# kursawe/OpticalFlow

Measured on AMD Instinct MI355X. Metric: frame-pairs/sec, higher is better.
Workload: dtype f64; 1 GPU; 1024x1024x256 synthetic translating texture (seed 1), speed_alpha=1, remodelling_alpha=1e4, rtol=1e-06, all 255 pairs solved to the stopping rule; frames_per_gpu=256, pairs_in_flight=255, levels=9, coarse_stencils=float8, vcycle_vectors=coarse_float32, w_cycle_level=1, w_cycle_visits=3, warm_start_stride=3, allgather=False, gather_chunks=1, converged=True

## Files before the change

opticalflow_amd/csrc/vof.hip:

```cpp
#include "vof_device.hpp"
#include "vof_sweep0r.hpp"
#include "vof_sweep0p.hpp"
#include "vof_direct.hpp"
#include "vof_boxflow.hpp"
#include "vof_boxsweep.hpp"
#include "vof_blursweep.hpp"
#include "vof_liushen.hpp"
#include "../../include/vof.h"

#include <fcntl.h>
#include <unistd.h>

#include <algorithm>
#include <atomic>
#include <chrono>
#include <cmath>
#include <condition_variable>
#include <cstdio>
#include <cstdlib>
#include <cstring>
#include <mutex>
#include <string>
#include <thread>
#include <vector>
// ... 72 lines not shown
    char* sw_aux = nullptr;
    size_t sw_aux_bytes = 0;
    bool bf_lds_set = false;
    bool bl_lds_set = false;
    bool ls_lds_set = false;
    double* tex_tab = nullptr;
    size_t tex_cap = 0;
    double* gm_V = nullptr;
    GmresState* gm_state = nullptr;
    double* gm_partials = nullptr;
    int* gm_cycle = nullptr;
    int gm_m = 0;
    long long gmres_pairs = 0;
    struct Alloc { void* raw; char* user; size_t bytes; const char* name; int line; };
    std::vector<Alloc> allocs;
    int c_bytes_per_point = 0;
    size_t bytes = 0;
    std::string err;
    const double* frames = nullptr;
    int npairs = 0;
    vof_params prm;
    int cfmt = 0;
    bool fused = true;
    bool fold_stored = false;
    bool direct_on = false;
    int dir_cap = 0;
    double *dir_T = nullptr, *dir_tabs = nullptr, *dir_W = nullptr, *dir_r = nullptr, *dir_y = nullptr, *dir_x = nullptr, *dir_t = nullptr;
    int *dir_ipiv = nullptr, *dir_info = nullptr;
    double *dir_R = nullptr, *dir_C = nullptr, *dir_D = nullptr;
    int dir_ld = 0;
    long long direct_pairs = 0;
    bool fuse_rr = true;
    bool fuse_b = true;
    long sweep0r_min_blocks = 512;
    int tail_first = -1;
    size_t tail_lds = 0;
    TailArgs tail;
    int tail_key[6] = {-9, -9, -9, -9, -9, -9};
    bool prof = false;
    int prof_kid = -1, prof_level = -1;
    std::vector<ProfRec> recs;
    std::vector<hipEvent_t> free_events;
    long long prof_dropped = 0;
    double prof_ms[VOF_K_COUNT][16];
    long long prof_n[VOF_K_COUNT][16];
    long long prof_units[VOF_K_COUNT][16];
    double prof_bytes[VOF_K_COUNT][16];
    double prof_moved[VOF_K_COUNT][16];
    int cur_units = 0;
    int dbg_sync = 0;
    long long dbg_seq = 0;
    std::string dbg_fault;
    int dbg_fd = -1;
    bool dbg_canary = false;
    bool dbg_alloc_log = false;
    bool dbg_poison = false;
    size_t part_per_pair = 0;
    vof_ctx* lane_parent = nullptr;
    int lane_lo = 0, lane_slots = 0;
    int dir_ok = -1;
    hipStream_t lane_stream[MAX_LANES] = {};
    hipEvent_t lane_ev[MAX_LANES][2] = {};
    hipEvent_t ev_fork = nullptr;
    hipEvent_t group_ev[MAX_LANES * MAX_LANE_GROUPS] = {};
};

// ... 262 lines not shown
    }
}

int pick_band_height(int rows, int nx, int units) {
    const long blocks128 = (long)nx * ((rows + 127) / 128) * std::max(1, units);
    const int cap = blocks128 < 768 ? 32 : (blocks128 < 1536 ? 64 : 128);
    const int nb = (rows + cap - 1) / cap;
    return std::max(2, (((rows + nb - 1) / nb + 1) / 2) * 2);
}

struct ApplyGrid { int TI, nblk; dim3 grid; };
ApplyGrid apply_grid(const vof_ctx* c, int np) {
    const Level& lv = c->L[0];
    int TI = pick_band_height(lv.ni, (lv.nj + AP_OUT - 1) / AP_OUT, c->cur_units);
    ApplyGrid g;
    g.TI = TI;
    g.grid = dim3((lv.nj + AP_OUT - 1) / AP_OUT, (lv.ni + TI - 1) / TI, np);
    g.nblk = g.grid.x * g.grid.y;
    return g;
}

template <typename XT, typename BT, typename YT>
void apply_fine_t(vof_ctx* c, const XT* x, const BT* b, YT* y, int mode, int np, const int* active,
                  const double* dotvec = nullptr, int want_yy = 0, YT* ycopy = nullptr) {
    Level& lv = c->L[0];
    const double bytes = (8.0 + 3.0 * sizeof(XT) + ((y ? 3.0 : 0.0) + (ycopy ? 3.0 : 0.0)) * sizeof(YT) + (mode ? 3.0 * sizeof(BT) : 0.0) +
                          (dotvec ? 24.0 : 0.0)) * lv.npts;
    Prof p(c, VOF_K_APPLY0, 0, bytes);
    ApplyGrid ag = apply_grid(c, np);
    double* part = (dotvec || want_yy) ? c->partials : nullptr;
    if (mode)
        k_stream_apply0<1, XT, BT, YT><<<ag.grid, AP_THREADS, 0, c->stream>>>(
            c->frames, frame_stride(c), c->Nj, lv.ni, lv.nj, ag.TI, c->prm.speed_alpha, c->prm.remodelling_alpha,
            c->prm.reference_quirks, x, b, y, dotvec, want_yy, part, ag.nblk, active, c->pp, ycopy);
    else
        k_stream_apply0<0, XT, BT, YT><<<ag.grid, AP_THREADS, 0, c->stream>>>(
            c->frames, frame_stride(c), c->Nj, lv.ni, lv.nj, ag.TI, c->prm.speed_alpha, c->prm.remodelling_alpha,
            c->prm.reference_quirks, x, b, y, dotvec, want_yy, part, ag.nblk, active, c->pp, ycopy);
}

template <typename VT>
void apply_stored_t(vof_ctx* c, int l, const VT* x, const VT* b, VT* y, int mode, int np, const int* active) {
    Level& lv = c->L[l];
    dim3 g = grid2d(lv.ni, lv.nj, np);
    Prof p(c, VOF_K_RESIDUAL, l, (coef_bytes(c, l) + (mode ? 9.0 : 6.0) * sizeof(VT)) * lv.npts);
    if (mode) CDISPATCH(c, l, (k_apply<CT, 1, VT><<<g, blk2d, 0, c->stream>>>((const CW*)lv.C, lv.ni, lv.nj, x, b, y, active)));
    else CDISPATCH(c, l, (k_apply<CT, 0, VT><<<g, blk2d, 0, c->stream>>>((const CW*)lv.C, lv.ni, lv.nj, x, b, y, active)));
}

template <typename VT>
void apply_level_t(vof_ctx* c, int l, const VT* x, const VT* b, VT* y, int mode, int np, const int* active) {
    if (l == 0 && c->L[0].C == nullptr) apply_fine_t<VT, VT, VT>(c, x, b, y, mode, np, active);
    else apply_stored_t<VT>(c, l, x, b, y, mode, np, active);
}

int krylov_apply(vof_ctx* c, const void* y, double* out, int np, const int* active, const double* dotvec = nullptr,
                 int want_yy = 0) {
    if (c->L[0].C) { apply_stored_t<double>(c, 0, (const double*)y, nullptr, out, 0, np, active); return 0; }
    if (c->vfloat || c->h32) apply_fine_t<float, double, double>(c, (const float*)y, nullptr, out, 0, np, active, dotvec, want_yy);
    else apply_fine_t<double, double, double>(c, (const double*)y, nullptr, out, 0, np, active, dotvec, want_yy);
    return (dotvec || want_yy) ? apply_grid(c, np).nblk : 0;
}
inline bool residual_copy_ok(const vof_ctx* c) { return !c->L[0].C; }
int residual_d(vof_ctx* c, const double* x, const double* b, double* out, int np, const int* active, int want_norm = 0,
               double* out2 = nullptr) {
    if (!out && !(want_norm && !c->L[0].C)) return 0;
    if (c->L[0].C) { apply_stored_t<double>(c, 0, x, b, out, 1, np, active); return 0; }
    apply_fine_t<double, double, double>(c, x, b, out, 1, np, active, nullptr, want_norm ? 1 : 0, out2);
    return want_norm ? apply_grid(c, np).nblk : 0;
}

template <typename VT>
void restrict_level_t(vof_ctx* c, int l, const VT* fine, VT* coarse, int np, const int* active) {
    Level &f = c->L[l], &k = c->L[l + 1];
    Prof p(c, VOF_K_RESTRICT, l, 3.0 * sizeof(VT) * (f.npts + k.npts));
    k_restrict<VT><<<grid2d(k.ni, k.nj, np), blk2d, 0, c->stream>>>(fine, f.ni, f.nj, coarse, k.ni, k.nj, active);
}

template <typename VT, typename CVT = VT>
void resrestrict_fine_t(vof_ctx* c, const VT* x, const VT* b, CVT* bc, int np, const int* active) {
    Level &f = c->L[0], &k = c->L[1];
    int TI = pick_band_height(f.ni, (k.nj + RR_CO - 1) / RR_CO, c->cur_units);
    dim3 g((k.nj + RR_CO - 1) / RR_CO, (k.ni + TI / 2 - 1) / (TI / 2), np);
    Prof p(c, VOF_K_APPLY0, 0, (8.0 + 6.0 * sizeof(VT)) * f.npts + 3.0 * sizeof(CVT) * k.npts);
    k_stream_resrestrict0<VT, VT, CVT><<<g, AP_THREADS, 0, c->stream>>>(
        c->frames, frame_stride(c), c->Nj, f.ni, f.nj, TI, c->prm.speed_alpha, c->prm.remodelling_alpha,
        c->prm.reference_quirks, x, b, bc, k.ni, k.nj, active, c->pp);
}

inline double resu_coef_bytes(const vof_ctx* c) {
    return c->cfmt == 3 ? 12.0 * 4 : (c->cfmt == 2 ? 18.5 * 4 : (c->cfmt == 1 ? 36.0 * 4 : 36.0 * 8));
}
template <typename VT>
void resrestrict_u_t(vof_ctx* c, int l, const VT* x_new, const VT* x_old, VT* bc, int np, const int* active) {
    Level &f = c->L[l], &k = c->L[l + 1];
    const double vs = sizeof(VT);
    const double algo = (coef_bytes(c, l) + 9.0 * vs) * f.npts + 3.0 * vs * (f.npts + k.npts);
    const double moved = (resu_coef_bytes(c) + (x_old ? 6.0 : 3.0) * vs) * f.npts + 3.0 * vs * k.npts;
    Prof p(c, VOF_K_RESIDUAL, l, algo, moved);
    dim3 g(1, (k.ni + BY - 1) / BY, np);
    CDISPATCH(c, l, {
        if (x_old) k_resrestrict_u<CT, VT, true><<<g, blk2d, 0, c->stream>>>((const CW*)f.C, f.ni, f.nj, x_new, x_old, bc, k.ni, k.nj, active);
// ... 900 lines not shown
        if (rq.table) {
            HIPCHK(hipMemcpyAsync(c->pp_buf, rq.table, (size_t)np * sizeof(PairParam), hipMemcpyHostToDevice, c->stream));
            c->pp = c->pp_buf;
        }
        if (rq.guess) {
            HIPCHK(hipMemcpyAsync(c->warm_src, rq.guess, (size_t)np * sizeof(int), hipMemcpyHostToDevice, c->stream));
            guess_src = c->warm_src;
        }
    }
    c->direct_on = rq.direct;
    struct MaxItGuard { vof_params& p; int saved; ~MaxItGuard() { p.max_iterations = saved; } } max_it_guard{c->prm, c->prm.max_iterations};
    constexpr int MG_ATTEMPT_CAP = 150;
    if (P.preconditioner == 2 && !c->direct_on && c->L.size() > 1 && P.max_iterations > MG_ATTEMPT_CAP && 3 * c->L[0].nj <= 3100 &&
        direct_ok_for_fallback(c))
        c->prm.max_iterations = MG_ATTEMPT_CAP;
    if (stats) HIPCHK(hipEventRecord(c->ev_batch[0], c->stream));
    c->vfloat = (P.vcycle_precision == 1 || P.vcycle_precision == 2) && c->fused && c->L.size() > 1 && !c->direct_on;
    c->vcoarse32 = P.vcycle_precision == 3 && !c->direct_on;
    c->h32 = false;
    if (c->direct_on) {
        if (np > c->dir_cap) { c->err = "batch larger than the direct preconditioner's buffers"; return -1; }
        c->frames = frames_dev;
        c->npairs = np;
        c->cur_units = np;
        if (int rc = direct_setup(c, np)) return rc;
        c->direct_pairs += np;
    } else if (int rc = setup_batch(c, frames_dev, np)) return rc;
    Level& f = c->L[0];
    const size_t len = 3 * f.npts;
    hipStream_t s = c->stream;
    double sx = P.delta_t / P.delta_x;
    const bool zero_guess = !guess_src && (P.initial_v_x == 0.0 && P.initial_v_y == 0.0 && P.initial_remodelling == 0.0);
    double* rh = c->krh;
    {
        Prof p(c, VOF_K_RHS, 0);
        k_rhs_norm<<<rgrid(c, np), RBLK, 0, s>>>(frames_dev, frame_stride(c), c->Nj, f.ni, f.nj, c->kb, zero_guess ? c->kr : nullptr,
                                                c->partials, c->pp);
    }
    { Prof p(c, VOF_K_VECTOR, 0); k_scalar<S_BNORM><<<np, 64, 0, s>>>(c->sc, c->partials, c->nblk, c->active, P.rtol, P.max_iterations); }
    int nb0 = c->nblk;
    if (zero_guess) {
        HIPCHK(hipMemsetAsync(c->kx, 0, (size_t)np * len * sizeof(double), s));
        rh = c->kb;
    } else {
        if (guess_src) {
            Prof p(c, VOF_K_VECTOR, 0, 16.0 * len);
            k_gather_guess<<<rgrid(c, np), RBLK, 0, s>>>(c->kx, c->warm_x, guess_src, len, f.npts, P.initial_v_x * sx, P.initial_v_y * sx,
                                                        P.initial_remodelling);
        } else {
            Prof p(c, VOF_K_VECTOR, 0); k_fill<<<dim3(c->nblk, np), 256, 0, s>>>(c->kx, f.npts, P.initial_v_x * sx, P.initial_v_y * sx, P.initial_remodelling);
        }
        const bool two = residual_copy_ok(c);
        nb0 = residual_d(c, c->kx, c->kb, c->kr, np, nullptr, 1, two ? c->krh : nullptr);
        if (!two) HIPCHK(hipMemcpyAsync(c->krh, c->kr, (size_t)np * len * sizeof(double), hipMemcpyDeviceToDevice, s));
    }
    if (!nb0) {
        Prof p(c, VOF_K_REDUCE, 0); k_dot2<<<rgrid(c, np), RBLK, 0, s>>>(c->kr, c->kr, nullptr, nullptr, len, c->partials, nullptr);
        nb0 = c->nblk;
    }
    { Prof p(c, VOF_K_VECTOR, 0); k_scalar<S_R0><<<np, 64, 0, s>>>(c->sc, c->partials, nb0, c->active, P.rtol, P.max_iterations); }

    const int bicg_limit = P.krylov_method == 1 ? 0 : (P.krylov_method == 2 ? std::min(P.max_iterations, P.fallback_after) : P.max_iterations);
    int it_total = 0;
    auto bicg_loop = [&](int limit) -> int {
    bool ran_on_r = false;
    for (int it = 0; it < limit; ++it, ++it_total) {
        HIPCHK(hipMemcpyAsync(c->h_active, c->active, np * sizeof(int), hipMemcpyDeviceToHost, s));
        HIPCHK(hipStreamSynchronize(s));
        int nact = 0;
        for (int k = 0; k < np; ++k) nact += c->h_active[k] != 0;
        if (nact == 0) break;
        if (it_total == AUTO_F64_AFTER) { if (P.vcycle_precision == 2) c->vfloat = false; c->vcoarse32 = false; }
        c->cur_units = nact;
        c->h32 = handoff32_ok(c);
        const int* act = c->active;
        void* vrhs_p = c->vfloat ? (void*)c->b32 : (void*)c->kp;
        void* vrhs_s = c->vfloat ? (void*)c->b32 : (void*)c->kr;
        const double vsz = (c->vfloat || c->h32) ? 4.0 : 8.0;
        const bool on_r = it == 0 && !c->vfloat;
        const bool fold_b = fold_b_usable(c);
        auto cycle_ok = [c](const CycleIO& io, const char* which) {
            if (io.failed) c->h32 = false;
            else if (io.bf_mode && !io.bf_done) c->err = std::string("folded vector update (") + which + "): not consumed by the cycle";
            else return true;
            return false;
        };
        CycleIO io_p, io_s;
        if (on_r) vrhs_p = (void*)c->kr;
        else if (fold_b && it > 0) {
            const double* p_old = (it == 1 && ran_on_r) ? rh : c->kp;
            io_p.bf = S0BSrc{c->kr, c->kv, p_old, c->kt, c->sc, nullptr};
            io_p.bf_mode = 2;
            std::swap(c->kp, c->kt);
// ... 17 lines not shown
            std::swap(c->kr, c->kt);
            vrhs_s = (void*)c->kr;
        } else {
        { Prof p(c, VOF_K_VECTOR, 0, 8.0 * len * 3 + (c->vfloat ? 4.0 * len : 0.0));
          VDISPATCH(c, (k_update_s<VT><<<rgrid(c, np), RBLK, 0, s>>>(c->kr, c->kv, len, c->sc, c->partials, act, c->vfloat ? (VT*)c->b32 : (VT*)nullptr))); }
        { Prof p(c, VOF_K_VECTOR, 0); k_scalar<S_S><<<np, 64, 0, s>>>(c->sc, c->partials, c->nblk, c->active, P.rtol, P.max_iterations); }
        { Prof p(c, VOF_K_VECTOR, 0);
          YDISPATCH(c, (k_fix_half<VT><<<dim3(64, np), RBLK, 0, s>>>(c->kx, (const VT*)c->ky, len, c->sc)));
          k_clear_half<<<(np + 255) / 256, 256, 0, s>>>(c->sc, np); }
        }
        io_s.trail = S0Trail{c->kt, c->kr, 1, c->partials};
        vcycle(c, &c->kz, vrhs_s, np, act, io_s);
        if (!cycle_ok(io_s, "s")) return -1;
        int nb2 = io_s.trail_nblk ? io_s.trail_nblk : krylov_apply(c, c->kz, c->kt, np, act, c->kr, 1);
        if (!nb2) { Prof p(c, VOF_K_REDUCE, 0, 16.0 * len); k_dot2<<<rgrid(c, np), RBLK, 0, s>>>(c->kt, c->kr, c->kt, c->kt, len, c->partials, act); nb2 = c->nblk; }
        { Prof p(c, VOF_K_VECTOR, 0); k_scalar<S_OMEGA><<<np, 64, 0, s>>>(c->sc, c->partials, nb2, c->active, P.rtol, P.max_iterations); }
        { Prof p(c, VOF_K_VECTOR, 0, 8.0 * len * 6 + 2.0 * vsz * len);
          YDISPATCH(c, (k_update_xr<VT><<<rgrid(c, np), RBLK, 0, s>>>(c->kx, (const VT*)c->ky, (const VT*)c->kz, c->kr, c->kt, rh, len, c->sc, c->partials, act))); }
        { Prof p(c, VOF_K_VECTOR, 0); k_scalar<S_R><<<np, 64, 0, s>>>(c->sc, c->partials, c->nblk, c->active, P.rtol, P.max_iterations); }
    }
    c->h32 = false;
    return 0;
    };
    if (int rc = bicg_loop(bicg_limit)) return rc;
    auto independent_residual = [&](bool keep) -> int {
        c->cur_units = np;
        int nb3 = keep ? 0 : residual_d(c, c->kx, c->kb, nullptr, np, nullptr, 1);
        if (!nb3) nb3 = residual_d(c, c->kx, c->kb, c->kt, np, nullptr, 1);
        if (!nb3) { Prof p(c, VOF_K_REDUCE, 0); k_dot2<<<rgrid(c, np), RBLK, 0, s>>>(c->kt, c->kt, nullptr, nullptr, len, c->partials, nullptr); nb3 = c->nblk; }
        { Prof p(c, VOF_K_VECTOR, 0); k_scalar<S_FINAL><<<np, 64, 0, s>>>(c->sc, c->partials, nb3, c->active, P.rtol, P.max_iterations); }
        HIPCHK(hipGetLastError());
        return 0;
    };
    if (int rc = independent_residual(false)) return rc;
    if (bicg_limit > 0) {
        for (int round = 0; round < 3; ++round) {
            { Prof p(c, VOF_K_VECTOR, 0); k_bicg_restart<<<(np + 63) / 64, 64, 0, s>>>(c->sc, c->active, np, P.max_iterations); }
            int nact = count_active(c, np);
            if (nact < 0) { c->err = "stream synchronize failed"; return -2; }
            if (nact == 0) break;
            if (int rc = independent_residual(true)) return rc;
            c->cur_units = nact;
            rh = c->krh;
            { Prof p(c, VOF_K_VECTOR, 0, 8.0 * len * 3);
              k_restart_vectors<<<rgrid(c, np), RBLK, 0, s>>>(c->kr, rh, c->kt, len, c->active); }
            if (int rc = bicg_loop(std::min(bicg_limit, 8))) return rc;
            if (int rc = independent_residual(false)) return rc;
        }
    }
    if (P.krylov_method != 0) {
        int handed_over = 0;
        if (int rc = gmres_phase(c, np, &handed_over)) return rc;
        if (handed_over)
            if (int rc = independent_residual(false)) return rc;
    }
    { Prof p(c, VOF_K_FINALIZE, 0);
      k_finalize_functionals<<<rgrid(c, np), RBLK, 0, s>>>(frames_dev, frame_stride(c), f.ni, f.nj, P.speed_alpha, P.remodelling_alpha,
                                                           P.reference_quirks, c->kx, P.delta_x / P.delta_t, rq.vx, rq.vy, rq.gm, rq.speed,
                                                           c->partials, c->pp);
      k_sum3<<<np, 64, 0, s>>>(c->partials, c->nblk, c->func3); }
    HIPCHK(hipGetLastError());
    if (stats) {
        HIPCHK(hipMemcpyAsync(c->h_sc, c->sc, np * sizeof(PairScalars), hipMemcpyDeviceToHost, s));
        HIPCHK(hipMemcpyAsync(c->h_func3, c->func3, np * 3 * sizeof(double), hipMemcpyDeviceToHost, s));
        HIPCHK(hipEventRecord(c->ev_batch[1], s));
        HIPCHK(hipStreamSynchronize(s));
        float batch_ms = 0.f;
        HIPCHK(hipEventElapsedTime(&batch_ms, c->ev_batch[0], c->ev_batch[1]));
        for (int k = 0; k < np; ++k) {
            const PairScalars& q = c->h_sc[k];
            stats[k].iterations = q.iterations;
            stats[k].relative_residual = q.bnorm2 > 0 ? std::sqrt(q.rnorm2 / q.bnorm2) : 0.0;
            stats[k].converged = (q.rnorm2 <= q.tol2) ? 1 : 0;
            stats[k].L1_functional = c->h_func3[3 * k];
            stats[k].speed_functional = c->h_func3[3 * k + 1];
            stats[k].remodelling_functional = c->h_func3[3 * k + 2];
            stats[k].batch_ms = batch_ms;
            stats[k].batch_pairs = np;
            stats[k].reserved = 0;
        }
    }
    return 0;
}

int check_params(vof_ctx* c, const vof_params* p) {
    if (!p) { c->err = "params is NULL"; return -1; }
    if (p->struct_size != sizeof(vof_params) || p->abi_version != VOF_VERSION) {
        char buf[256];
        snprintf(buf, sizeof buf, "vof_params ABI mismatch: caller has struct_size %u / version %u, library has %zu / %d "
                 "(fill the struct with vof_default_params(p, sizeof *p) of the matching include/vof.h)",
                 p->struct_size, p->abi_version, sizeof(vof_params), VOF_VERSION);
        c->err = buf;
        return -4;
// ... 131 lines not shown
    for (hipEvent_t e : c->group_ev) if (e) hipEventDestroy(e);
    if (c->own_stream && c->stream) hipStreamDestroy(c->stream);
    delete c;
}

static int create_impl(vof_ctx* c, int device_id, int n_i, int n_j, int B, void* stream) {
    if (n_i < 4 || n_j < 4) { c->err = "image must be at least 4x4 (the mirror boundary rows need N >= 4)"; return -1; }
    if (B < 1) { c->err = "max_pairs_in_flight must be >= 1"; return -1; }
    int ndev = 0;
    HIPCHK(hipGetDeviceCount(&ndev));
    if (device_id < 0 || device_id >= ndev) { c->err = "no such HIP device"; return -1; }
    HIPCHK(hipSetDevice(device_id));
    c->device = device_id;
    c->Ni = n_i; c->Nj = n_j; c->B = B;
    if (stream) { c->stream = (hipStream_t)stream; c->own_stream = false; }
    else { HIPCHK(hipStreamCreate(&c->stream)); c->own_stream = true; }
    memset(c->prof_ms, 0, sizeof c->prof_ms);
    memset(c->prof_n, 0, sizeof c->prof_n);
    memset(c->prof_units, 0, sizeof c->prof_units);
    memset(c->prof_bytes, 0, sizeof c->prof_bytes);
    memset(c->prof_moved, 0, sizeof c->prof_moved);
    vof_default_params(&c->prm, sizeof c->prm);
    if (const char* e = getenv("VOF_DEBUG_SYNC")) c->dbg_sync = atoi(e);
    if (const char* e = getenv("VOF_DEBUG_CANARY")) c->dbg_canary = e[0] != '0';
    if (const char* e = getenv("VOF_DEBUG_ALLOC_LOG")) c->dbg_alloc_log = e[0] != '0';
    if (const char* e = getenv("VOF_DEBUG_POISON")) c->dbg_poison = e[0] != '0';
    if (c->dbg_sync)
        if (const char* e = getenv("VOF_DEBUG_SYNC_FILE")) c->dbg_fd = open(e, O_WRONLY | O_CREAT, 0644);
    if (const char* e = getenv("VOF_FOLD_STORED")) c->fold_stored = e[0] != '0';
    if (const char* e = getenv("VOF_L0_HANDOFF")) c->l0_handoff = e[0] != '0';
    if (const char* e = getenv("VOF_SWEEP0R_MIN_BLOCKS")) c->sweep0r_min_blocks = atol(e);
    if (const char* e = getenv("VOF_FUSE_B")) c->fuse_b = e[0] != '0';
    if (const char* e = getenv("VOF_FUSE_RR")) c->fuse_rr = e[0] != '0';
    Level l0; l0.ni = n_i - 2; l0.nj = n_j - 2; l0.npts = (size_t)l0.ni * l0.nj;
    c->L.push_back(l0);
    while (std::max(c->L.back().ni, c->L.back().nj) > COARSEST_MAX) {
        Level k; k.ni = (c->L.back().ni + 1) / 2; k.nj = (c->L.back().nj + 1) / 2; k.npts = (size_t)k.ni * k.nj;
        c->L.push_back(k);
    }
    int nl = (int)c->L.size();
    if (nl > 16) { c->err = "too many levels"; return -1; }
    size_t len0 = 3 * l0.npts;
    for (double** v : {&c->kx, &c->kb, &c->kr, &c->krh, &c->kp, &c->kv, &c->kt, &c->ky, &c->kz})
        if (int rc = dev_alloc(c, v, (size_t)B * len0)) return rc;
    for (int l = 0; l < nl; ++l) {
        Level& lv = c->L[l];
        auto valloc = [&](void** q) { double* t = nullptr; int rc = dev_alloc(c, &t, (size_t)B * 3 * lv.npts); *q = t; return rc; };
        if (l + 1 < nl && l > 0) if (int rc = valloc(&lv.r)) return rc;
        if (l + 1 < nl) if (int rc = valloc(&lv.x2)) return rc;
        if (l > 0) {
            if (int rc = valloc(&lv.x)) return rc;
            if (int rc = valloc(&lv.b)) return rc;
        }
        if (nl == 1) {
            double* C = nullptr;
            if (int rc = dev_alloc(c, &C, (size_t)B * 81 * CLay(lv.ni, lv.nj).plane)) return rc;
            lv.C = C;
        }
    }
    if (int rc = ensure_stencil_storage(c, vof_params_default_coarse_precision())) return rc;
    c->nd = 3 * (int)c->L.back().npts;
    {
        int first = -1;
        for (int l = 1; l < nl; ++l) {
            const CLay lay(c->L[l].ni, c->L[l].nj);
            if (c->L[l].npts <= (size_t)TAIL_MAX_PTS && lay.sub <= (size_t)TAIL_MAX_SUB) { first = l; break; }
// ... 11 lines not shown
            }
            c->tail.ro = off; off += 3 * (int)c->L[first].npts;
            c->tail.nl = nl - first;
            c->tail.nd = c->nd;
            c->tail.n_ops = 0;
            c->tail_lds = (size_t)off * sizeof(double);
            if (c->tail_lds <= (size_t)150 * 1024) {
                c->tail_first = first;
                const int lds = (int)c->tail_lds;
                HIPCHK(hipFuncSetAttribute((const void*)k_tail_cycle<CoefB16, double>, hipFuncAttributeMaxDynamicSharedMemorySize, lds));
                HIPCHK(hipFuncSetAttribute((const void*)k_tail_cycle<CoefB16, float>, hipFuncAttributeMaxDynamicSharedMemorySize, lds));
                HIPCHK(hipFuncSetAttribute((const void*)k_tail_cycle<CoefF8, double>, hipFuncAttributeMaxDynamicSharedMemorySize, lds));
                HIPCHK(hipFuncSetAttribute((const void*)k_tail_cycle<CoefF8, float>, hipFuncAttributeMaxDynamicSharedMemorySize, lds));
                HIPCHK(hipFuncSetAttribute((const void*)k_tail_cycle<float, double>, hipFuncAttributeMaxDynamicSharedMemorySize, lds));
                HIPCHK(hipFuncSetAttribute((const void*)k_tail_cycle<float, float>, hipFuncAttributeMaxDynamicSharedMemorySize, lds));
                HIPCHK(hipFuncSetAttribute((const void*)k_tail_cycle<double, double>, hipFuncAttributeMaxDynamicSharedMemorySize, lds));
                HIPCHK(hipFuncSetAttribute((const void*)k_tail_cycle<double, float>, hipFuncAttributeMaxDynamicSharedMemorySize, lds));
            }
        }
    }
    if (int rc = dev_alloc(c, &c->W, (size_t)B * c->nd * 2 * c->nd)) return rc;
    if (int rc = dev_alloc(c, &c->invT, (size_t)B * c->nd * c->nd)) return rc;
    {
        const int lds = 18 * s0_row_bytes(8) + 9 * (S0_W / 2 + 2) * 8;
        HIPCHK(hipFuncSetAttribute((const void*)k_sweep0m<2, true, false, 1>, hipFuncAttributeMaxDynamicSharedMemorySize, lds));
        HIPCHK(hipFuncSetAttribute((const void*)k_sweep0m<2, false, false, 1>, hipFuncAttributeMaxDynamicSharedMemorySize, lds));
        HIPCHK(hipFuncSetAttribute((const void*)k_sweep0m<1, true, false, 1>, hipFuncAttributeMaxDynamicSharedMemorySize, lds));
        HIPCHK(hipFuncSetAttribute((const void*)k_sweep0m<1, false, false, 1>, hipFuncAttributeMaxDynamicSharedMemorySize, lds));
    }
    c->nblk = (int)std::min<size_t>(256, std::max<size_t>(1, (len0 + 4 * RBLK - 1) / (4 * RBLK)));
    {
        int nblk_apply = ((l0.nj + AP_OUT - 1) / AP_OUT) * ((l0.ni + 31) / 32 + 1);
        nblk_apply = std::max(nblk_apply, ((l0.nj + 99) / 100) * ((l0.ni + 1 + 31) / 32 + 1));
        c->part_per_pair = (size_t)3 * std::max(c->nblk, nblk_apply);
        if (int rc = dev_alloc(c, &c->partials, (size_t)B * c->part_per_pair)) return rc;
    }
    if (int rc = dev_alloc(c, &c->sc, (size_t)B)) return rc;
    if (int rc = dev_alloc(c, &c->active, (size_t)B)) return rc;
    if (int rc = dev_alloc(c, &c->func3, (size_t)B * 3)) return rc;
    HIPCHK(hipHostMalloc((void**)&c->h_active, B * sizeof(int)));
    HIPCHK(hipHostMalloc((void**)&c->h_sc, B * sizeof(PairScalars)));
    HIPCHK(hipHostMalloc((void**)&c->h_func3, B * 3 * sizeof(double)));
    for (int i = 0; i < 2; ++i) HIPCHK(hipEventCreate(&c->ev_batch[i]));
    return 0;
}

int vof_create(vof_ctx** out, int device_id, int n_i, int n_j, int max_pairs_in_flight, void* stream) {
    if (!out) { g_create_error = "out is NULL"; return -1; }
    *out = nullptr;
    vof_ctx* c = new (std::nothrow) vof_ctx();
    if (!c) { g_create_error = "out of host memory"; return -1; }
    int rc = create_impl(c, device_id, n_i, n_j, max_pairs_in_flight, stream);
    if (rc) {
        g_create_error = c->err;
        vof_destroy(c);
        return rc;
    }
    *out = c;
    return 0;
}

}

namespace {

double lanes_min_pixels() {
    double mpix = 16.0;
// ... 1844 lines not shown
```

opticalflow_amd/csrc/vof_device.hpp:

```cpp
#pragma once
#include <hip/hip_runtime.h>
#include <stdint.h>
#include <type_traits>

namespace vof {

constexpr int BX = 64;
constexpr int BY = 4;
constexpr int NT = BX * BY;

struct PairScalars {
    double rho, alpha, omega, beta;
    double bnorm2, rnorm2;
    double tol2;
    int iterations;
    int converged;
    int breakdown;
    int halfstep;
};

struct PairParam {
    double alpha, beta;
    int frame;
    int out;
// ... 2764 lines not shown
    };

    for (int s = s_first; s <= s_last; ++s) {
        const int e = 2 * s;
        if (e >= e_lo && e <= e_hi) step(std::false_type{}, e);
        else step(std::true_type{}, e);
        ringL = wrapB(ringL + 2 * RSB);
        rowC = wrapB(rowC + 2 * RSB);
        gL += 2 * (long long)nj; gW += 2 * (long long)nj; gB += 2 * (long long)nj; gI += 2 * (long long)Nj;
        if (TRAIL) { gT += 2 * (long long)nj; rowT = wrapB(rowT + 2 * RSB); }
        __syncthreads();
    }
    if (TRAIL) {
        double* red = reinterpret_cast<double*>(ring);
        const double a0 = wave_sum(ts0), a1 = wave_sum(ts1);
        if (lane == 0) { red[2 * wave] = a0; red[2 * wave + 1] = a1; }
        __syncthreads();
        if (threadIdx.x == 0 && tr.partials) {
            const int nblk = nx * ny, blk = by * nx + bx;
            double* pp = tr.partials + ((size_t)pair * 3) * nblk + blk;
            double q0 = 0.0, q1 = 0.0;
#pragma unroll
            for (int w2 = 0; w2 < NW; ++w2) { q0 += red[2 * w2]; q1 += red[2 * w2 + 1]; }
            pp[0] = q0;
            if (tr.dotvec && tr.want_vv) pp[nblk] = q1;
        }
    }
}

constexpr int AP_OUT = 128, AP_W = 132, AP_THREADS = 256;
constexpr int AP_RING = 6;
__device__ __forceinline__ int ap_slot(int row) { return (row + 64 * AP_RING) % AP_RING; }

template <int MODE, typename XT, typename BT, typename YT>
__global__ __launch_bounds__(AP_THREADS) void k_stream_apply0(
    const double* __restrict__ frames, size_t frame_stride, int Nj, int ni, int nj, int TI, double alpha, double beta,
    int quirks, const XT* __restrict__ x, const BT* __restrict__ b, YT* __restrict__ y,
    const double* __restrict__ dotvec, int want_yy, double* __restrict__ partials, int nblk,
    const int* __restrict__ active, const PairParam* __restrict__ pp, YT* __restrict__ ycopy) {
    __shared__ XT xs[AP_RING * 3 * AP_W];
    __shared__ double im[AP_RING * AP_W];
    __shared__ double red[2][AP_THREADS / 64];
    const int pair = blockIdx.z;
    if (active && !active[pair]) return;
    int fidx = pair;
    if (pp) { alpha = pp[pair].alpha; beta = pp[pair].beta; fidx = pp[pair].frame; }
    const int tid = threadIdx.x;
    const int half = __builtin_amdgcn_readfirstlane(tid >> 7);
    const int col = tid & 127;
    const int q0 = blockIdx.x * AP_OUT, p0 = blockIdx.y * TI;
    const int q = q0 + col;
    const bool col_ok = q < nj;
    const size_t npts = (size_t)ni * nj, off = (size_t)pair * 3 * npts;
    const XT* xp = x + off;
    const double* img = frames + (size_t)fidx * frame_stride;
    const bool oL = q - 1 < 0, oR = q + 1 >= nj;
    const int cC = col + 1, cL = oL ? col + 2 : col, cR = oR ? col : col + 2;
    double s0 = 0.0, s1 = 0.0;
    const int nsteps = TI / 2;
    BT bn0 = (BT)0, bn1 = (BT)0, bn2 = (BT)0;
    double dn0 = 0.0, dn1 = 0.0, dn2 = 0.0;
    for (int s = -2; s < nsteps; ++s) {
        const int r = 2 * s;
        const BT bc0 = bn0, bc1 = bn1, bc2 = bn2;
        const double dc0 = dn0, dc1 = dn1, dc2 = dn2;
        const int rl = r + 3 + half, pl = p0 + rl;
        const bool row_ld = rl <= TI && pl >= 0 && pl < ni;
        const bool irow_ld = rl <= TI && pl + 1 >= 0 && pl + 1 <= ni + 1;
        XT l0 = (XT)0, l1 = (XT)0, l2 = (XT)0, h0 = (XT)0, h1 = (XT)0, h2 = (XT)0;
        double li0 = 0.0, li1 = 0.0;
        if (row_ld) {
            const XT* xr = xp + (size_t)pl * nj;
            if (col_ok) { l0 = xr[q]; l1 = xr[npts + q]; l2 = xr[2 * npts + q]; }
            const int qh = (col == 0) ? q0 - 1 : q0 + AP_OUT;
            if ((col == 0 || col == 127) && qh >= 0 && qh < nj) { h0 = xr[qh]; h1 = xr[npts + qh]; h2 = xr[2 * npts + qh]; }
        }
        if (irow_ld) {
            const double* ir = img + (size_t)(pl + 1) * Nj;
            if (q0 + col <= nj + 1) li0 = ir[q0 + col];
            if (col < 2 && q0 + 128 + col <= nj + 1) li1 = ir[q0 + 128 + col];
        }
        {
            const int rcn = r + 2 + half, pn = p0 + rcn;
            if (s + 1 >= 0 && rcn < TI && pn < ni && col_ok) {
                const size_t idn = (size_t)pn * nj + q;
                if (MODE == 1) { bn0 = b[off + idn]; bn1 = b[off + npts + idn]; bn2 = b[off + 2 * npts + idn]; }
                if (dotvec) { dn0 = dotvec[off + idn]; dn1 = dotvec[off + npts + idn]; dn2 = dotvec[off + 2 * npts + idn]; }
            }
        }
        const int rc = r + half, p = p0 + rc;
        if (s >= 0 && rc < TI && p < ni && col_ok) {
            const bool oU = p - 1 < 0, oD = p + 1 >= ni;
            const int sU = ap_slot(rc - 1), sC = ap_slot(rc), sD = ap_slot(rc + 1);
            const double* i0 = im + sU * AP_W;
            const double* i1 = im + sC * AP_W;
            const double* i2 = im + sD * AP_W;
            double imm = i0[col], im0 = i0[col + 1], imp = i0[col + 2];
            double i0m = i1[col], i00 = i1[col + 1], i0p = i1[col + 2];
            double ipm = i2[col], ip0 = i2[col + 1], ipp = i2[col + 2];
            PixCoef k;
            k.P = i00;
            k.Dx = (ip0 - im0) / 2;
            k.Dy = quirks ? k.Dx : (i0p - i0m) / 2;
            k.Dxx = ip0 + im0 - 2 * i00;
            k.Dyy = i0p + i0m - 2 * i00;
            k.Dxy = (ipp - ipm - imp + imm) / 4;
            const XT* ru = xs + (oU ? sD : sU) * 3 * AP_W;
            const XT* rcn = xs + sC * 3 * AP_W;
            const XT* rd = xs + (oD ? sU : sD) * 3 * AP_W;
            const double sUL = (oU && oL) ? 2.0 : 1.0, sUR = (oU && oR) ? 2.0 : 1.0;
            const double sDL = (oD && oL) ? 2.0 : 1.0, sDR = (oD && oR) ? 2.0 : 1.0;
            Nbr n;
            n.u[0] = sUL * (double)ru[cL]; n.w[0] = sUL * (double)ru[AP_W + cL];
            n.u[1] = (double)ru[cC];       n.w[1] = (double)ru[AP_W + cC];       n.g[1] = (double)ru[2 * AP_W + cC];
            n.u[2] = sUR * (double)ru[cR]; n.w[2] = sUR * (double)ru[AP_W + cR];
            n.u[3] = (double)rcn[cL];      n.w[3] = (double)rcn[AP_W + cL];      n.g[3] = (double)rcn[2 * AP_W + cL];
            n.u[4] = (double)rcn[cC];      n.w[4] = (double)rcn[AP_W + cC];      n.g[4] = (double)rcn[2 * AP_W + cC];
            n.u[5] = (double)rcn[cR];      n.w[5] = (double)rcn[AP_W + cR];      n.g[5] = (double)rcn[2 * AP_W + cR];
            n.u[6] = sDL * (double)rd[cL]; n.w[6] = sDL * (double)rd[AP_W + cL];
            n.u[7] = (double)rd[cC];       n.w[7] = (double)rd[AP_W + cC];       n.g[7] = (double)rd[2 * AP_W + cC];
            n.u[8] = sDR * (double)rd[cR]; n.w[8] = sDR * (double)rd[AP_W + cR];
            double y0, y1, y2;
            offdiag0(k, alpha, beta, n, y0, y1, y2);
            const double P = k.P;
            y0 += (P * (k.Dxx - 2 * P) - 4 * alpha) * n.u[4] + P * k.Dxy * n.w[4];
            y1 += (P * (k.Dyy - 2 * P) - 4 * alpha) * n.w[4] + P * k.Dxy * n.u[4];
            y2 += (-1 - 4 * beta) * n.g[4] + k.Dx * n.u[4] + k.Dy * n.w[4];
            const size_t idx = (size_t)p * nj + q;
            if (MODE == 1) {
                y0 = (double)bc0 - y0;
                y1 = (double)bc1 - y1;
                y2 = (double)bc2 - y2;
            }
            if (y) {
                y[off + idx] = (YT)y0;
                y[off + npts + idx] = (YT)y1;
                y[off + 2 * npts + idx] = (YT)y2;
            }
            if (ycopy) {
                ycopy[off + idx] = (YT)y0;
                ycopy[off + npts + idx] = (YT)y1;
                ycopy[off + 2 * npts + idx] = (YT)y2;
            }
            if (dotvec) {
                s0 += y0 * dc0 + y1 * dc1 + y2 * dc2;
                if (want_yy) s1 += y0 * y0 + y1 * y1 + y2 * y2;
            } else if (want_yy) {
                s0 += y0 * y0 + y1 * y1 + y2 * y2;
            }
        }
        if (rl <= TI) {
            const int sl = ap_slot(rl);
            XT* xr = xs + sl * 3 * AP_W;
            xr[col + 1] = l0; xr[AP_W + col + 1] = l1; xr[2 * AP_W + col + 1] = l2;
            if (col == 0 || col == 127) {
                const int ch = (col == 0) ? 0 : AP_OUT + 1;
                xr[ch] = h0; xr[AP_W + ch] = h1; xr[2 * AP_W + ch] = h2;
            }
            double* ir = im + sl * AP_W;
            ir[col] = li0;
            if (col < 2) ir[128 + col] = li1;
        }
        __syncthreads();
    }
    if (partials && (dotvec || want_yy)) {
        s0 = wave_sum(s0);
        s1 = wave_sum(s1);
        const int lane = tid & 63, wv = tid >> 6;
        if (lane == 0) { red[0][wv] = s0; red[1][wv] = s1; }
        __syncthreads();
        if (tid == 0) {
            double t0 = 0, t1 = 0;
            for (int i = 0; i < AP_THREADS / 64; ++i) { t0 += red[0][i]; t1 += red[1][i]; }
            const int blk = blockIdx.y * gridDim.x + blockIdx.x;
            double* pp = partials + ((size_t)pair * 3) * nblk + blk;
            pp[0] = t0;
            if (dotvec && want_yy) pp[nblk] = t1;
        }
    }
}

constexpr int RR_CO = 63;

template <typename XT, typename BT, typename CT2>
__global__ __launch_bounds__(AP_THREADS) void k_stream_resrestrict0(
    const double* __restrict__ frames, size_t frame_stride, int Nj, int ni, int nj, int TI, double alpha, double beta,
    int quirks, const XT* __restrict__ x, const BT* __restrict__ b, CT2* __restrict__ bc, int nci, int ncj,
    const int* __restrict__ active, const PairParam* __restrict__ pp) {
    __shared__ XT xs[AP_RING * 3 * AP_W];
    __shared__ double im[AP_RING * AP_W];
    __shared__ double rs[AP_RING * 3 * 128];
    const int pair = blockIdx.z;
    if (active && !active[pair]) return;
    int fidx = pair;
    if (pp) { alpha = pp[pair].alpha; beta = pp[pair].beta; fidx = pp[pair].frame; }
    const int tid = threadIdx.x;
    const int half = __builtin_amdgcn_readfirstlane(tid >> 7);
    const int col = tid & 127;
    const int q0 = blockIdx.x * (2 * RR_CO) - 1;
    const int p0 = blockIdx.y * TI - 1;
    const int q = q0 + col;
    const bool col_ok = q >= 0 && q < nj;
    const size_t npts = (size_t)ni * nj, off = (size_t)pair * 3 * npts;
    const XT* xp = x + off;
    const double* img = frames + (size_t)fidx * frame_stride;
    const bool oL = q - 1 < 0, oR = q + 1 >= nj;
    const int cC = col + 1, cL = oL ? col + 2 : col, cR = oR ? col : col + 2;
    const int ef = tid / RR_CO, em = tid % RR_CO;
    const int ecq = blockIdx.x * RR_CO + em;
    const bool e_on = tid < 3 * RR_CO && ecq < ncj;
// ... 397 lines not shown
```

Before: 1348 frame-pairs/s.

## Fuse solve prologue and epilogue into streaming fine-level apply kernel

Adds two new modes of the streaming fine-grid apply kernel. The prologue mode gathers the warm-start guess, computes the right-hand side from the frame pair, writes x and b, and computes the initial residual plus both norms in one pass. The epilogue mode computes the final residual norm, the energy functionals and the output velocity and remodelling fields (including boundary copies) in one pass. This replaces separate rhs, gather, residual and finalize kernels over the full-resolution data, cutting repeated global memory traffic and launches. It costs larger partial buffers, more kernel template complexity, and a changed occupancy hint for the epilogue.

```diff
diff --git a/opticalflow_amd/csrc/vof.hip b/opticalflow_amd/csrc/vof.hip
--- a/opticalflow_amd/csrc/vof.hip
+++ b/opticalflow_amd/csrc/vof.hip
@@ -128,6 +128,7 @@
     long long direct_pairs = 0;
     bool fuse_rr = true;
     bool fuse_b = true;
+    int fused_ends = 3;
     long sweep0r_min_blocks = 512;
     int tail_first = -1;
     size_t tail_lds = 0;
@@ -456,11 +457,11 @@
     if (mode)
         k_stream_apply0<1, XT, BT, YT><<<ag.grid, AP_THREADS, 0, c->stream>>>(
             c->frames, frame_stride(c), c->Nj, lv.ni, lv.nj, ag.TI, c->prm.speed_alpha, c->prm.remodelling_alpha,
-            c->prm.reference_quirks, x, b, y, dotvec, want_yy, part, ag.nblk, active, c->pp, ycopy);
+            c->prm.reference_quirks, x, b, y, dotvec, want_yy, part, ag.nblk, active, c->pp, ycopy, ApEnds{});
     else
         k_stream_apply0<0, XT, BT, YT><<<ag.grid, AP_THREADS, 0, c->stream>>>(
             c->frames, frame_stride(c), c->Nj, lv.ni, lv.nj, ag.TI, c->prm.speed_alpha, c->prm.remodelling_alpha,
-            c->prm.reference_quirks, x, b, y, dotvec, want_yy, part, ag.nblk, active, c->pp, ycopy);
+            c->prm.reference_quirks, x, b, y, dotvec, want_yy, part, ag.nblk, active, c->pp, ycopy, ApEnds{});
 }
 
 template <typename VT>
@@ -492,6 +493,30 @@
     if (c->L[0].C) { apply_stored_t<double>(c, 0, x, b, out, 1, np, active); return 0; }
     apply_fine_t<double, double, double>(c, x, b, out, 1, np, active, nullptr, want_norm ? 1 : 0, out2);
     return want_norm ? apply_grid(c, np).nblk : 0;
+}
+
+int fused_prologue(vof_ctx* c, const int* src, double c0, double c1, double c2, int np) {
+    Level& lv = c->L[0];
+    Prof p(c, VOF_K_RHS, 0, (src ? 192.0 : 168.0) * lv.npts, (src ? 136.0 : 112.0) * lv.npts);
+    ApplyGrid ag = apply_grid(c, np);
+    ApEnds e{};
+    e.saved = c->warm_x; e.src = src; e.c0 = c0; e.c1 = c1; e.c2 = c2; e.xo = c->kx; e.bo = c->kb;
+    k_stream_apply0<2, double, double, double><<<ag.grid, AP_THREADS, 0, c->stream>>>(
+        c->frames, frame_stride(c), c->Nj, lv.ni, lv.nj, ag.TI, c->prm.speed_alpha, c->prm.remodelling_alpha,
+        c->prm.reference_quirks, nullptr, nullptr, c->kr, nullptr, 0, c->partials, ag.nblk, nullptr, c->pp, c->krh, e);
+    return ag.nblk;
+}
+int fused_epilogue(vof_ctx* c, double* vx, double* vy, double* gm, double* speed, double* fpart, int np) {
+    Level& lv = c->L[0];
+    const double out = speed ? 32.0 : 24.0;
+    Prof p(c, VOF_K_FINALIZE, 0, (96.0 + out) * lv.npts, (64.0 + out) * lv.npts);
+    ApplyGrid ag = apply_grid(c, np);
+    ApEnds e{};
+    e.vscale = c->prm.delta_x / c->prm.delta_t; e.vx = vx; e.vy = vy; e.gm = gm; e.speed = speed; e.fpartials = fpart;
+    k_stream_apply0<3, double, double, double><<<ag.grid, AP_THREADS, 0, c->stream>>>(
+        c->frames, frame_stride(c), c->Nj, lv.ni, lv.nj, ag.TI, c->prm.speed_alpha, c->prm.remodelling_alpha,
+        c->prm.reference_quirks, c->kx, c->kb, nullptr, nullptr, 1, c->partials, ag.nblk, nullptr, c->pp, nullptr, e);
+    return ag.nblk;
 }
 
 template <typename VT>
@@ -1458,17 +1483,24 @@
     double sx = P.delta_t / P.delta_x;
     const bool zero_guess = !guess_src && (P.initial_v_x == 0.0 && P.initial_v_y == 0.0 && P.initial_remodelling == 0.0);
     double* rh = c->krh;
-    {
+    const bool fuse_pro = (c->fused_ends & 1) && !zero_guess && residual_copy_ok(c) && !c->direct_on;
+    int nbb = c->nblk;
+    int nb0 = c->nblk;
+    const double* part_r0 = c->partials;
+    if (fuse_pro) {
+        c->cur_units = np;
+        nbb = nb0 = fused_prologue(c, guess_src, P.initial_v_x * sx, P.initial_v_y * sx, P.initial_remodelling, np);
+        part_r0 = c->partials + nb0;
+    } else {
         Prof p(c, VOF_K_RHS, 0);
         k_rhs_norm<<<rgrid(c, np), RBLK, 0, s>>>(frames_dev, frame_stride(c), c->Nj, f.ni, f.nj, c->kb, zero_guess ? c->kr : nullptr,
                                                 c->partials, c->pp);
     }
-    { Prof p(c, VOF_K_VECTOR, 0); k_scalar<S_BNORM><<<np, 64, 0, s>>>(c->sc, c->partials, c->nblk, c->active, P.rtol, P.max_iterations); }
-    int nb0 = c->nblk;
+    { Prof p(c, VOF_K_VECTOR, 0); k_scalar<S_BNORM><<<np, 64, 0, s>>>(c->sc, c->partials, nbb, c->active, P.rtol, P.max_iterations); }
     if (zero_guess) {
         HIPCHK(hipMemsetAsync(c->kx, 0, (size_t)np * len * sizeof(double), s));
         rh = c->kb;
-    } else {
+    } else if (!fuse_pro) {
         if (guess_src) {
             Prof p(c, VOF_K_VECTOR, 0, 16.0 * len);
             k_gather_guess<<<rgrid(c, np), RBLK, 0, s>>>(c->kx, c->warm_x, guess_src, len, f.npts, P.initial_v_x * sx, P.initial_v_y * sx,
@@ -1479,12 +1511,12 @@
         const bool two = residual_copy_ok(c);
         nb0 = residual_d(c, c->kx, c->kb, c->kr, np, nullptr, 1, two ? c->krh : nullptr);
         if (!two) HIPCHK(hipMemcpyAsync(c->krh, c->kr, (size_t)np * len * sizeof(double), hipMemcpyDeviceToDevice, s));
-    }
-    if (!nb0) {
-        Prof p(c, VOF_K_REDUCE, 0); k_dot2<<<rgrid(c, np), RBLK, 0, s>>>(c->kr, c->kr, nullptr, nullptr, len, c->partials, nullptr);
-        nb0 = c->nblk;
-    }
-    { Prof p(c, VOF_K_VECTOR, 0); k_scalar<S_R0><<<np, 64, 0, s>>>(c->sc, c->partials, nb0, c->active, P.rtol, P.max_iterations); }
+        if (!nb0) {
+            Prof p(c, VOF_K_REDUCE, 0); k_dot2<<<rgrid(c, np), RBLK, 0, s>>>(c->kr, c->kr, nullptr, nullptr, len, c->partials, nullptr);
+            nb0 = c->nblk;
+        }
+    }
+    { Prof p(c, VOF_K_VECTOR, 0); k_scalar<S_R0><<<np, 64, 0, s>>>(c->sc, part_r0, nb0, c->active, P.rtol, P.max_iterations); }
 
     const int bicg_limit = P.krylov_method == 1 ? 0 : (P.krylov_method == 2 ? std::min(P.max_iterations, P.fallback_after) : P.max_iterations);
     int it_total = 0;
@@ -1568,13 +1600,23 @@
         HIPCHK(hipGetLastError());
         return 0;
     };
-    if (int rc = independent_residual(false)) return rc;
+    bool finalized = false;
+    if ((c->fused_ends & 2) && residual_copy_ok(c)) {
+        c->cur_units = np;
+        double* fpart = c->partials + (size_t)np * 3 * apply_grid(c, np).nblk;
+        const int nb3 = fused_epilogue(c, rq.vx, rq.vy, rq.gm, rq.speed, fpart, np);
+        { Prof p(c, VOF_K_VECTOR, 0); k_scalar<S_FINAL><<<np, 64, 0, s>>>(c->sc, c->partials, nb3, c->active, P.rtol, P.max_iterations); }
+        { Prof p(c, VOF_K_FINALIZE, 0); k_sum3<<<np, 64, 0, s>>>(fpart, nb3, c->func3); }
+        HIPCHK(hipGetLastError());
+        finalized = true;
+    } else if (int rc = independent_residual(false)) return rc;
     if (bicg_limit > 0) {
         for (int round = 0; round < 3; ++round) {
             { Prof p(c, VOF_K_VECTOR, 0); k_bicg_restart<<<(np + 63) / 64, 64, 0, s>>>(c->sc, c->active, np, P.max_iterations); }
             int nact = count_active(c, np);
             if (nact < 0) { c->err = "stream synchronize failed"; return -2; }
             if (nact == 0) break;
+            finalized = false;
             if (int rc = independent_residual(true)) return rc;
             c->cur_units = nact;
             rh = c->krh;
@@ -1587,14 +1629,18 @@
     if (P.krylov_method != 0) {
         int handed_over = 0;
         if (int rc = gmres_phase(c, np, &handed_over)) return rc;
-        if (handed_over)
+        if (handed_over) {
+            finalized = false;
             if (int rc = independent_residual(false)) return rc;
-    }
-    { Prof p(c, VOF_K_FINALIZE, 0);
-      k_finalize_functionals<<<rgrid(c, np), RBLK, 0, s>>>(frames_dev, frame_stride(c), f.ni, f.nj, P.speed_alpha, P.remodelling_alpha,
-                                                           P.reference_quirks, c->kx, P.delta_x / P.delta_t, rq.vx, rq.vy, rq.gm, rq.speed,
-                                                           c->partials, c->pp);
-      k_sum3<<<np, 64, 0, s>>>(c->partials, c->nblk, c->func3); }
+        }
+    }
+    if (!finalized) {
+        Prof p(c, VOF_K_FINALIZE, 0);
+        k_finalize_functionals<<<rgrid(c, np), RBLK, 0, s>>>(frames_dev, frame_stride(c), f.ni, f.nj, P.speed_alpha, P.remodelling_alpha,
+                                                             P.reference_quirks, c->kx, P.delta_x / P.delta_t, rq.vx, rq.vy, rq.gm, rq.speed,
+                                                             c->partials, c->pp);
+        k_sum3<<<np, 64, 0, s>>>(c->partials, c->nblk, c->func3);
+    }
     HIPCHK(hipGetLastError());
     if (stats) {
         HIPCHK(hipMemcpyAsync(c->h_sc, c->sc, np * sizeof(PairScalars), hipMemcpyDeviceToHost, s));
@@ -1792,6 +1838,7 @@
     if (const char* e = getenv("VOF_SWEEP0R_MIN_BLOCKS")) c->sweep0r_min_blocks = atol(e);
     if (const char* e = getenv("VOF_FUSE_B")) c->fuse_b = e[0] != '0';
     if (const char* e = getenv("VOF_FUSE_RR")) c->fuse_rr = e[0] != '0';
+    if (const char* e = getenv("VOF_FUSED_ENDS")) { const int v = atoi(e); if (v >= 0 && v <= 3) c->fused_ends = v; }
     Level l0; l0.ni = n_i - 2; l0.nj = n_j - 2; l0.npts = (size_t)l0.ni * l0.nj;
     c->L.push_back(l0);
     while (std::max(c->L.back().ni, c->L.back().nj) > COARSEST_MAX) {
@@ -1869,7 +1916,7 @@
     {
         int nblk_apply = ((l0.nj + AP_OUT - 1) / AP_OUT) * ((l0.ni + 31) / 32 + 1);
         nblk_apply = std::max(nblk_apply, ((l0.nj + 99) / 100) * ((l0.ni + 1 + 31) / 32 + 1));
-        c->part_per_pair = (size_t)3 * std::max(c->nblk, nblk_apply);
+        c->part_per_pair = (size_t)6 * std::max(c->nblk, nblk_apply);
         if (int rc = dev_alloc(c, &c->partials, (size_t)B * c->part_per_pair)) return rc;
     }
     if (int rc = dev_alloc(c, &c->sc, (size_t)B)) return rc;
diff --git a/opticalflow_amd/csrc/vof_device.hpp b/opticalflow_amd/csrc/vof_device.hpp
--- a/opticalflow_amd/csrc/vof_device.hpp
+++ b/opticalflow_amd/csrc/vof_device.hpp
@@ -2820,15 +2820,27 @@
 constexpr int AP_RING = 6;
 __device__ __forceinline__ int ap_slot(int row) { return (row + 64 * AP_RING) % AP_RING; }
 
+struct ApEnds {
+    const double* saved; const int* src; double c0, c1, c2;
+    double* xo; double* bo;
+    double vscale; double *vx, *vy, *gm, *speed;
+    double* fpartials;
+};
+
 template <int MODE, typename XT, typename BT, typename YT>
-__global__ __launch_bounds__(AP_THREADS) void k_stream_apply0(
+__global__ __launch_bounds__(AP_THREADS) __attribute__((amdgpu_waves_per_eu(MODE == 3 ? 3 : 1))) void k_stream_apply0(
     const double* __restrict__ frames, size_t frame_stride, int Nj, int ni, int nj, int TI, double alpha, double beta,
     int quirks, const XT* __restrict__ x, const BT* __restrict__ b, YT* __restrict__ y,
     const double* __restrict__ dotvec, int want_yy, double* __restrict__ partials, int nblk,
-    const int* __restrict__ active, const PairParam* __restrict__ pp, YT* __restrict__ ycopy) {
+    const int* __restrict__ active, const PairParam* __restrict__ pp, YT* __restrict__ ycopy, ApEnds e) {
     __shared__ XT xs[AP_RING * 3 * AP_W];
     __shared__ double im[AP_RING * AP_W];
-    __shared__ double red[2][AP_THREADS / 64];
+    __shared__ double jm[MODE == 2 ? AP_RING * AP_W : 1];
+    __shared__ double red[MODE == 3 ? 5 : 2][AP_THREADS / 64];
+    const double* const dotv = MODE >= 2 ? nullptr : dotvec;
+    const int wyy = MODE == 3 ? 1 : want_yy;
+    YT* const yo = MODE == 3 ? nullptr : y;
+    YT* const yc = MODE == 3 ? nullptr : ycopy;
     const int pair = blockIdx.z;
     if (active && !active[pair]) return;
     int fidx = pair;
@@ -2842,6 +2854,13 @@
     const size_t npts = (size_t)ni * nj, off = (size_t)pair * 3 * npts;
     const XT* xp = x + off;
     const double* img = frames + (size_t)fidx * frame_stride;
+    if (MODE == 2) {
+        const int sp = e.src ? e.src[pair] : -1;
+        xp = sp >= 0 ? (const XT*)(e.saved + (size_t)sp * 3 * npts) : nullptr;
+    }
+    const size_t obase = MODE == 3 ? (size_t)(pp ? pp[pair].out : pair) * (size_t)(ni + 2) * Nj : 0;
+    double f0 = 0.0, f1 = 0.0, f2 = 0.0;
+    double jn = 0.0;
     const bool oL = q - 1 < 0, oR = q + 1 >= nj;
     const int cC = col + 1, cL = oL ? col + 2 : col, cR = oR ? col : col + 2;
     double s0 = 0.0, s1 = 0.0;
@@ -2850,30 +2869,47 @@
     double dn0 = 0.0, dn1 = 0.0, dn2 = 0.0;
     for (int s = -2; s < nsteps; ++s) {
         const int r = 2 * s;
-        const BT bc0 = bn0, bc1 = bn1, bc2 = bn2;
+        BT bc0 = bn0, bc1 = bn1, bc2 = bn2;
+        const double jc = jn;
         const double dc0 = dn0, dc1 = dn1, dc2 = dn2;
         const int rl = r + 3 + half, pl = p0 + rl;
         const bool row_ld = rl <= TI && pl >= 0 && pl < ni;
         const bool irow_ld = rl <= TI && pl + 1 >= 0 && pl + 1 <= ni + 1;
         XT l0 = (XT)0, l1 = (XT)0, l2 = (XT)0, h0 = (XT)0, h1 = (XT)0, h2 = (XT)0;
-        double li0 = 0.0, li1 = 0.0;
+        double li0 = 0.0, li1 = 0.0, lj0 = 0.0, lj1 = 0.0;
         if (row_ld) {
-            const XT* xr = xp + (size_t)pl * nj;
-            if (col_ok) { l0 = xr[q]; l1 = xr[npts + q]; l2 = xr[2 * npts + q]; }
             const int qh = (col == 0) ? q0 - 1 : q0 + AP_OUT;
-            if ((col == 0 || col == 127) && qh >= 0 && qh < nj) { h0 = xr[qh]; h1 = xr[npts + qh]; h2 = xr[2 * npts + qh]; }
+            const bool halo = (col == 0 || col == 127) && qh >= 0 && qh < nj;
+            if (MODE == 2 && !xp) {
+                if (col_ok) { l0 = (XT)e.c0; l1 = (XT)e.c1; l2 = (XT)e.c2; }
+                if (halo) { h0 = (XT)e.c0; h1 = (XT)e.c1; h2 = (XT)e.c2; }
+            } else {
+                const XT* xr = xp + (size_t)pl * nj;
+                if (col_ok) { l0 = xr[q]; l1 = xr[npts + q]; l2 = xr[2 * npts + q]; }
+                if (halo) { h0 = xr[qh]; h1 = xr[npts + qh]; h2 = xr[2 * npts + qh]; }
+            }
+            if (MODE == 2 && rl >= 0 && rl < TI && col_ok) {
+                const size_t idl = off + (size_t)pl * nj + q;
+                e.xo[idl] = (double)l0; e.xo[npts + idl] = (double)l1; e.xo[2 * npts + idl] = (double)l2;
+            }
         }
         if (irow_ld) {
             const double* ir = img + (size_t)(pl + 1) * Nj;
             if (q0 + col <= nj + 1) li0 = ir[q0 + col];
             if (col < 2 && q0 + 128 + col <= nj + 1) li1 = ir[q0 + 128 + col];
+            if (MODE == 2) {
+                const double* jr = ir + frame_stride;
+                if (q0 + col <= nj + 1) lj0 = jr[q0 + col];
+                if (col < 2 && q0 + 128 + col <= nj + 1) lj1 = jr[q0 + 128 + col];
+            }
         }
         {
             const int rcn = r + 2 + half, pn = p0 + rcn;
             if (s + 1 >= 0 && rcn < TI && pn < ni && col_ok) {
                 const size_t idn = (size_t)pn * nj + q;
                 if (MODE == 1) { bn0 = b[off + idn]; bn1 = b[off + npts + idn]; bn2 = b[off + 2 * npts + idn]; }
-                if (dotvec) { dn0 = dotvec[off + idn]; dn1 = dotvec[off + npts + idn]; dn2 = dotvec[off + 2 * npts + idn]; }
+                if (dotv) { dn0 = dotv[off + idn]; dn1 = dotv[off + npts + idn]; dn2 = dotv[off + 2 * npts + idn]; }
+                if (MODE == 3) jn = img[frame_stride + (size_t)(pn + 1) * Nj + q + 1];
             }
         }
         const int rc = r + half, p = p0 + rc;
@@ -2915,26 +2951,76 @@
             y1 += (P * (k.Dyy - 2 * P) - 4 * alpha) * n.w[4] + P * k.Dxy * n.u[4];
             y2 += (-1 - 4 * beta) * n.g[4] + k.Dx * n.u[4] + k.Dy * n.w[4];
             const size_t idx = (size_t)p * nj + q;
-            if (MODE == 1) {
+            if (MODE == 2) {
+                const double* j0 = jm + sU * AP_W;
+                const double* j1 = jm + sC * AP_W;
+                const double* j2 = jm + sD * AP_W;
+                const double dxt = (j2[col + 1] - j0[col + 1] - ip0 + im0) / 2;
+                const double dyt = (j1[col + 2] - j1[col] - i0p + i0m) / 2;
+                const double dt = j1[col + 1] - i00;
+                {
+#pragma clang fp contract(off)
+                    bc0 = -P * dxt; bc1 = -P * dyt; bc2 = -dt;
+                }
+                e.bo[off + idx] = bc0; e.bo[off + npts + idx] = bc1; e.bo[off + 2 * npts + idx] = bc2;
+                s0 += (double)bc0 * bc0 + (double)bc1 * bc1 + (double)bc2 * bc2;
+            }
+            if (MODE == 3) {
+                const double u0 = n.u[4], w0 = n.w[4], g0 = n.g[4];
+                const double dt = jc - k.P;
+                const double dux = (n.u[7] - n.u[1]) / 2, dwx = (n.w[7] - n.w[1]) / 2, dgx = (n.g[7] - n.g[1]) / 2;
+                const double duy = quirks ? dux : (n.u[5] - n.u[3]) / 2;
+                const double dwy = quirks ? dwx : (n.w[5] - n.w[3]) / 2;
+                const double dgy = quirks ? dgx : (n.g[5] - n.g[3]) / 2;
+                const double ee = dt + u0 * k.Dx + w0 * k.Dy + k.P * dux + k.P * dwy - g0;
+                f0 += ee * ee;
+                f1 += dux * dux + duy * duy + dwx * dwx + dwy * dwy;
+                f2 += dgx * dgx + dgy * dgy;
+            }
+            if (MODE == 3) { bc0 = b[off + idx]; bc1 = b[off + npts + idx]; bc2 = b[off + 2 * npts + idx]; }
+            if (MODE >= 1) {
                 y0 = (double)bc0 - y0;
                 y1 = (double)bc1 - y1;
                 y2 = (double)bc2 - y2;
             }
-            if (y) {
-                y[off + idx] = (YT)y0;
-                y[off + npts + idx] = (YT)y1;
-                y[off + 2 * npts + idx] = (YT)y2;
-            }
-            if (ycopy) {
-                ycopy[off + idx] = (YT)y0;
-                ycopy[off + npts + idx] = (YT)y1;
-                ycopy[off + 2 * npts + idx] = (YT)y2;
-            }
-            if (dotvec) {
+            if (yo) {
+                yo[off + idx] = (YT)y0;
+                yo[off + npts + idx] = (YT)y1;
+                yo[off + 2 * npts + idx] = (YT)y2;
+            }
+            if (yc) {
+                yc[off + idx] = (YT)y0;
+                yc[off + npts + idx] = (YT)y1;
+                yc[off + 2 * npts + idx] = (YT)y2;
+            }
+            if (MODE == 2) {
+                s1 += y0 * y0 + y1 * y1 + y2 * y2;
+            } else if (dotv) {
                 s0 += y0 * dc0 + y1 * dc1 + y2 * dc2;
-                if (want_yy) s1 += y0 * y0 + y1 * y1 + y2 * y2;
-            } else if (want_yy) {
+                if (wyy) s1 += y0 * y0 + y1 * y1 + y2 * y2;
+            } else if (wyy) {
                 s0 += y0 * y0 + y1 * y1 + y2 * y2;
+            }
+            if (MODE == 3) {
+                const double u0 = n.u[4], w0 = n.w[4], g0 = n.g[4];
+                const double u = u0 * e.vscale, w = w0 * e.vscale;
+                const double sp = e.speed ? sqrt(u * u + w * w) : 0.0;
+                auto put = [&](int i, int j) {
+                    const size_t t = obase + (size_t)i * Nj + j;
+                    e.vx[t] = u; e.vy[t] = w; e.gm[t] = g0;
+                    if (e.speed) e.speed[t] = sp;
+                };
+                const int iA = p == 1 ? 0 : -1, iB = p == ni - 2 ? ni + 1 : -1;
+                const int jA = q == 1 ? 0 : -1, jB = q == nj - 2 ? nj + 1 : -1;
+                put(p + 1, q + 1);
+                if ((iA & iB & jA & jB) >= 0) {
+                    const int ri[3] = {p + 1, iA, iB}, cj[3] = {q + 1, jA, jB};
+#pragma unroll
+                    for (int a = 0; a < 3; ++a)
+#pragma unroll
+                        for (int c2 = 0; c2 < 3; ++c2)
+                            if (a + c2 > 0 && ri[a] >= 0 && cj[c2] >= 0) put(ri[a], cj[c2]);
+                }
             }
         }
         if (rl <= TI) {
@@ -2948,14 +3034,23 @@
             double* ir = im + sl * AP_W;
             ir[col] = li0;
             if (col < 2) ir[128 + col] = li1;
+            if (MODE == 2) {
+                double* jr = jm + sl * AP_W;
+                jr[col] = lj0;
+                if (col < 2) jr[128 + col] = lj1;
+            }
         }
         __syncthreads();
     }
-    if (partials && (dotvec || want_yy)) {
+    if (partials && (dotv || wyy || MODE == 2)) {
         s0 = wave_sum(s0);
         s1 = wave_sum(s1);
         const int lane = tid & 63, wv = tid >> 6;
         if (lane == 0) { red[0][wv] = s0; red[1][wv] = s1; }
+        if (MODE == 3) {
+            f0 = wave_sum(f0); f1 = wave_sum(f1); f2 = wave_sum(f2);
+            if (lane == 0) { red[2][wv] = f0; red[3][wv] = f1; red[4][wv] = f2; }
+        }
         __syncthreads();
         if (tid == 0) {
             double t0 = 0, t1 = 0;
@@ -2963,7 +3058,13 @@
             const int blk = blockIdx.y * gridDim.x + blockIdx.x;
             double* pp = partials + ((size_t)pair * 3) * nblk + blk;
             pp[0] = t0;
-            if (dotvec && want_yy) pp[nblk] = t1;
+            if ((dotv && wyy) || MODE == 2) pp[nblk] = t1;
+            if (MODE == 3) {
+                double g0 = 0, g1 = 0, g2 = 0;
+                for (int i = 0; i < AP_THREADS / 64; ++i) { g0 += red[2][i]; g1 += red[3][i]; g2 += red[4][i]; }
+                double* fp = e.fpartials + ((size_t)pair * 3) * nblk + blk;
+                fp[0] = g0; fp[nblk] = alpha * g1; fp[2 * (size_t)nblk] = beta * g2;
+            }
         }
     }
 }
```

Result: faster. 1380 frame-pairs/s, median of 6 (+2.4%).
